# yakvrz/minesweeper-ppo

Hardware: AMD Instinct MI355X
Metric: env steps/sec (16x16x40, N envs) + PPO updates/sec at 1/2/4/8 MI355X (higher is better)
Workload: dtype u8/u64 board bits -> f32 obs; 1 GPU; board step 16x16x40, 4096 envs per GPU (BASELINE configs[1]); board=16x16x40, envs_per_gpu=4096, envs_total=4096, tape=0, parallelism=env-shard x1, no collective, obs_ring_slots=13

## Files before the change

### minesweeper-ppo_amd/csrc/msenv.hip

```cpp
#include <hip/hip_ext.h>
#include <hip/hip_runtime.h>

#include <stddef.h>
#include <stdint.h>
#include <stdio.h>
#include <stdlib.h>
#include <string.h>

#include <new>
#include <type_traits>
#include <vector>

#include "../../include/msenv.h"
#include "../../include/msenv_debug.h"
#include "msenv_internal.h"

namespace {

constexpr int kWave = 64;
constexpr int kMaxH = 64;
constexpr int kMaxW = 62;

struct alignas(16) EnvMeta {
  uint64_t st_hi, st_lo, inc_hi, inc_lo;
  uint32_t has32, uinteger;
  int32_t step_count;
  uint32_t flags;
};
static_assert(sizeof(EnvMeta) == 48, "EnvMeta layout");

struct KParams {
  const void* actions;
  float* obs;
  uint8_t* mask;
  float* reward;
  uint8_t* done;
  int32_t* step;
  int32_t* last_new;
  double* frac;
  int8_t* outcome;
  EnvMeta* meta;
  uint64_t* mine_words;
  uint64_t* rev_words;
  int64_t n;
  int32_t H, W, K, guarantee;
  int32_t actions_i32;
  double win_reward, loss_reward, step_penalty;
  const uint64_t* jump;
  uint64_t* diag;
  uint32_t dbg_flags;
  uint8_t* codes;
};

__device__ __forceinline__ int lane_id() { return __builtin_amdgcn_mbcnt_hi(~0u, __builtin_amdgcn_mbcnt_lo(~0u, 0u)); }

__device__ __forceinline__ uint32_t rfl(uint32_t x) { return (uint32_t)__builtin_amdgcn_readfirstlane((int)x); }
__device__ __forceinline__ uint64_t rfl64(uint64_t x) {
  return ((uint64_t)rfl((uint32_t)(x >> 32)) << 32) | rfl((uint32_t)x);
}

template <int CTRL>
__device__ __forceinline__ uint32_t dpp32(uint32_t v) {
  return (uint32_t)__builtin_amdgcn_update_dpp(0, (int)v, CTRL, 0xf, 0xf, true);
}
__device__ __forceinline__ uint64_t wave_shr1(uint64_t v) {
  return ((uint64_t)dpp32<0x138>((uint32_t)(v >> 32)) << 32) | dpp32<0x138>((uint32_t)v);
}
__device__ __forceinline__ uint64_t wave_shl1(uint64_t v) {
  return ((uint64_t)dpp32<0x130>((uint32_t)(v >> 32)) << 32) | dpp32<0x130>((uint32_t)v);
}
__device__ __forceinline__ uint32_t readlane32(uint32_t v, int l) {
  return (uint32_t)__builtin_amdgcn_readlane((int)v, l);
}
__device__ __forceinline__ uint64_t readlane64(uint64_t v, int l) {
  return ((uint64_t)readlane32((uint32_t)(v >> 32), l) << 32) | readlane32((uint32_t)v, l);
}
__device__ __forceinline__ void wave_sync() {
  __builtin_amdgcn_fence(__ATOMIC_RELEASE, "wavefront");
  __builtin_amdgcn_wave_barrier();
  __builtin_amdgcn_fence(__ATOMIC_ACQUIRE, "wavefront");
}
__device__ __forceinline__ uint32_t wave_sum(uint32_t v) {
  v += dpp32<0x111>(v);
  v += dpp32<0x112>(v);
  v += dpp32<0x114>(v);
  v += dpp32<0x118>(v);
  return readlane32(v, 15) + readlane32(v, 31) + readlane32(v, 47) + readlane32(v, 63);
}

#ifndef MS_OBS_STORE
#define MS_OBS_STORE 2
#endif
static_assert(MS_OBS_STORE >= 0 && MS_OBS_STORE <= 2, "MS_OBS_STORE: 0 plain, 1 nt, 2 write-through");
constexpr int kObsStore = MS_OBS_STORE;
constexpr int kObsStorePackedStep = kObsStore == 2 ? 1 : kObsStore;
constexpr int kObsStorePackedRun = kObsStore == 2 ? 0 : kObsStore;
typedef float f32x4_t __attribute__((ext_vector_type(4)));

template <int FORM = kObsStore>
__device__ __forceinline__ void store_plane4(float4* p, float4 v) {
  if constexpr (FORM == 1) {
    f32x4_t x = {v.x, v.y, v.z, v.w};
    __builtin_nontemporal_store(x, reinterpret_cast<f32x4_t*>(p));
  } else if constexpr (FORM == 2) {
    f32x4_t x = {v.x, v.y, v.z, v.w};
// ... 635 lines not shown
      }
      rev |= Fr;
      newly = (uint32_t)__popcll(Fr);
    }
  }
  const uint32_t packed = wave_sum(((uint32_t)__popcll(rev) << 16) | newly);
  total_rev = packed >> 16;
  newly = packed & 0xffffu;
  if (!cell_rev && outcome != MS_OUTCOME_LOSS && (int)total_rev >= A - p.K) {
    done = true;
    outcome = MS_OUTCOME_WIN;
  }
}

__device__ __forceinline__ void store_aux(const KParams& p, int64_t idx, int lane, double reward, bool done,
                                          int32_t step_count, uint32_t newly, uint32_t total_rev, int outcome, int A) {
  typedef __attribute__((address_space(1))) uint32_t gu32;
  typedef __attribute__((address_space(1))) uint8_t gu8;
  const uint64_t pr = rfl64((uint64_t)p.reward), ps = rfl64((uint64_t)p.step), pl = rfl64((uint64_t)p.last_new);
  const uint64_t pd = rfl64((uint64_t)p.done), po = rfl64((uint64_t)p.outcome);
  gu32* d4 = (gu32*)(lane == 0 ? pr : (lane == 1 ? ps : pl));
  const uint32_t v4 = lane == 0 ? __float_as_uint((float)reward) : (lane == 1 ? (uint32_t)step_count : newly);
  if (lane < 3 && d4) d4[idx] = v4;
  gu8* d1 = (gu8*)(lane == 0 ? pd : po);
  const uint8_t v1 = lane == 0 ? (uint8_t)(done ? 1 : 0) : (uint8_t)(int8_t)outcome;
  if (lane < 2 && d1) d1[idx] = v1;
  if (lane == 0 && p.frac) p.frac[idx] = (double)total_rev / (double)(A > 1 ? A : 1);
}

__device__ __forceinline__ void store_meta(EnvMeta* mp, const Pcg& rng, int32_t step_count, bool fc, int lane) {
  if (lane == 0) {
    *reinterpret_cast<ulonglong2*>(&mp->st_hi) = make_ulonglong2(rng.hi, rng.lo);
    *reinterpret_cast<uint4*>(&mp->has32) =
        make_uint4(rng.has32, rng.uinteger, (uint32_t)step_count, fc ? 1u : 0u);
  }
}

template <int H_, int W_, int EPW>
__global__ __launch_bounds__(64 * EPW) void k_step(EnvMeta* meta0, uint64_t* mine_words0, uint64_t* rev_words0,
                                                   const void* actions0, const uint64_t* jump0, int64_t n0,
                                                   int32_t actions_i32_0, int32_t K0, KParams p) {
  __shared__ uint64_t sR_all[EPW][kWave];
  __shared__ uint64_t sM_all[EPW][kWave + 2];
  __shared__ uint32_t sTab_all[EPW][(H_ && W_) ? H_ * W_ : kMaxH * kMaxW];
  const int lane = lane_id();
  const int wv = (EPW == 1) ? 0 : (int)rfl(threadIdx.x >> 6);
  const int64_t env_raw = (int64_t)blockIdx.x * EPW + wv;
  const bool live = env_raw < n0;
  const int64_t env = live ? env_raw : n0 - 1;
  uint64_t* sR = sR_all[wv];
  uint64_t* sM = sM_all[wv];
  uint32_t* sTab = sTab_all[wv];
  STAMP(0);
  const Geo<H_, W_> g(p.H, p.W);
  const int A = g.A(), NW = g.NW();

  EnvMeta* mp = meta0 + env;
  uint64_t* mwords = mine_words0 + env * NW;
  uint64_t* rwords = rev_words0 + env * NW;
  uint64_t mine = load_row(mwords, g, lane);
  uint64_t rev = load_row(rwords, g, lane);
  uint64_t J[4] = {0ull, 0ull, 0ull, 0ull};
  if (lane < K0) {
    const ulonglong2* e = reinterpret_cast<const ulonglong2*>(jump0 + 4 * lane);
    const ulonglong2 a0 = e[0], a1 = e[1];
    J[0] = a0.x;
    J[1] = a0.y;
    J[2] = a1.x;
    J[3] = a1.y;
  }
  Pcg rng;
  rng.hi = rfl64(mp->st_hi);
  rng.lo = rfl64(mp->st_lo);
  rng.ihi = rfl64(mp->inc_hi);
  rng.ilo = rfl64(mp->inc_lo);
  rng.has32 = rfl(mp->has32);
  rng.uinteger = rfl(mp->uinteger);
  int32_t step_count = (int32_t)rfl((uint32_t)mp->step_count);
  bool fc = (rfl(mp->flags) & 1u) != 0;
  const uint32_t* ap = reinterpret_cast<const uint32_t*>(actions0);
  const int64_t aw = actions_i32_0 ? env : 2 * env;
  const uint32_t a_lo = ap[aw], a_hi = ap[actions_i32_0 ? aw : aw + 1];
  int64_t a = actions_i32_0 ? (int64_t)(int32_t)a_lo : (int64_t)(((uint64_t)a_hi << 32) | a_lo);
  a = (int64_t)rfl64((uint64_t)a);
  int64_t cell64 = a % A;
  if (cell64 < 0) cell64 += A;
  const int cell = (int)cell64;
  if (!live) return;
  STAMP(1);

  double reward = 0.0;
  bool done = false;
  int outcome = MS_OUTCOME_NONE;
  uint32_t newly = 0, total_rev = 0;
  bool mines_changed = false;
  board_click(rng, mine, rev, fc, cell, p, J, sTab, sR, g, lane, done, outcome, newly, total_rev, mines_changed,
              env);
  STAMP(3);
  if (outcome == MS_OUTCOME_LOSS) reward += p.loss_reward;
  if (outcome == MS_OUTCOME_WIN) reward += p.win_reward;
  reward -= p.step_penalty;
  step_count += 1;

  store_aux(p, env, lane, reward, done, step_count, newly, total_rev, outcome, A);
  if (done) {
    mine = 0ull;
    rev = 0ull;
    fc = false;
    step_count = 0;
    mines_changed = true;
  }
  STAMP(4);

  if (p.obs || p.mask || p.codes) {
    stage_rows(sR, sM, rev, mine, g, lane);
    emit_obs(p.obs ? p.obs + env * 10 * A : nullptr, p.mask ? p.mask + env * A : nullptr,
             p.codes ? p.codes + env * A : nullptr, sR, sM, fc, g, lane, reinterpret_cast<uint8_t*>(sTab));
  }
  store_meta(mp, rng, step_count, fc, lane);
  if (mines_changed) store_rows(mwords, mine, sR, g, lane);
  store_rows(rwords, rev, sR, g, lane);
  STAMP(5);
}


template <int B>
__device__ __forceinline__ float ub2f(uint32_t w) {
  return (float)((w >> (8 * B)) & 0xffu);
}

__device__ __forceinline__ uint32_t row_shr1(uint32_t v) { return dpp32<0x111>(v); }
__device__ __forceinline__ uint32_t row_shl1(uint32_t v) { return dpp32<0x101>(v); }
template <int LPB>
__device__ __forceinline__ int board_base(int lane) { return lane & (64 - LPB); }
template <int LPB>
__device__ __forceinline__ uint32_t board_sum(uint32_t v, int lane) {
  v += dpp32<0x128>(v);
  v += dpp32<0x124>(v);
  v += dpp32<0x122>(v);
  v += dpp32<0x121>(v);
  if (LPB == 32) v += bperm(v, lane ^ 16);
  return v;
}
template <int LPB>
__device__ __forceinline__ bool board_any(bool v, int lane) {
  constexpr uint64_t M = LPB == 64 ? ~0ull : ((1ull << LPB) - 1ull);
  return ((__ballot(v) >> board_base<LPB>(lane)) & M) != 0ull;
}
template <int LPB>
__device__ __forceinline__ uint32_t board_read(uint32_t v, int lane, int r) {
  return bperm(v, board_base<LPB>(lane) | (r & 15));
}
template <int LPB>
__device__ __forceinline__ uint64_t board_read64(uint64_t v, int lane, int r) {
  return ((uint64_t)board_read<LPB>((uint32_t)(v >> 32), lane, r) << 32) | board_read<LPB>((uint32_t)v, lane, r);
}

template <int H_, int W_>
__device__ __forceinline__ uint32_t set_row(uint64_t s0, uint64_t s1, int r, const Geo<H_, W_>& g) {
  if (r >= g.H) return 0u;
  const int s = r * g.W;
  const uint64_t v = s >= 64 ? (s1 >> (s - 64)) : ((s0 >> s) | (s ? (s1 << (64 - s)) : 0ull));
  return (uint32_t)(v & g.rowmask());
}
__device__ __forceinline__ bool set_has(uint64_t s0, uint64_t s1, uint32_t c) {
  return (((c < 64u) ? s0 : s1) >> (c & 63u)) & 1ull;
}
__device__ __forceinline__ void set_add(uint64_t& s0, uint64_t& s1, uint32_t c) {
  const uint64_t bit = 1ull << (c & 63u);
  if (c < 64u) s0 |= bit;
  else s1 |= bit;
// ... 433 lines not shown
    const bool f = bperm(fc ? 1u : 0u, 16 * b) != 0u;
    const uint32_t m1 = m << 1, up1 = mu << 1, dn1 = md << 1;
    uint32_t cnt[4], rb[4];
#pragma unroll
    for (int e = 0; e < 4; ++e) {
      const int c = c0 + e;
      cnt[e] = (uint32_t)__popc((up1 >> c) & 7u) + (uint32_t)__popc((dn1 >> c) & 7u) + ((m1 >> c) & 1u) +
               ((m1 >> (c + 2)) & 1u);
      rb[e] = (rv >> c) & 1u;
    }
    if (ob) {
      float4* o4 = reinterpret_cast<float4*>(ob + (size_t)b * 10 * A) + lane;
#pragma unroll
      for (int ch = 0; ch < 10; ++ch) {
        float v[4];
#pragma unroll
        for (int e = 0; e < 4; ++e)
          v[e] = ch == 0 ? (float)rb[e] : ((f && rb[e] && cnt[e] + 1u == (uint32_t)ch) ? 1.f : 0.f);
        store_plane4(o4 + ch * (A / 4), make_float4(v[0], v[1], v[2], v[3]));
      }
    }
    if (mb)
      reinterpret_cast<uint32_t*>(mb + (size_t)b * A)[lane] =
          (rb[0] ^ 1u) | ((rb[1] ^ 1u) << 8) | ((rb[2] ^ 1u) << 16) | ((rb[3] ^ 1u) << 24);
  }
}

template <int H_, int W_, int BPW, int LPB, class Lds>
__device__ __forceinline__ void pk_store_state(EnvMeta* mp, uint64_t* mwords, uint64_t* rwords, const Pcg& rng,
                                               int32_t step_count, bool fc, uint32_t mine, uint32_t rev,
                                               bool mines_changed, bool live, Lds& S, int lane) {
  constexpr int RPW = 64 / W_;
  constexpr int NW = (H_ + RPW - 1) / RPW;
  const int r = lane & (LPB - 1);
  store_meta(mp, rng, step_count, fc, live ? r : 1);
  const int rb = board_base<LPB>(lane);
  S.row[lane] = mine;
  S.rev[lane] = rev;
  wave_sync();
  if (live && r < NW) {
    uint64_t am = 0ull, ar_ = 0ull;
#pragma unroll
    for (int k = 0; k < RPW; ++k)
      if (r * RPW + k < H_) {
        am |= (uint64_t)S.row[rb + r * RPW + k] << (k * W_);
        ar_ |= (uint64_t)S.rev[rb + r * RPW + k] << (k * W_);
      }
    if (mines_changed) mwords[r] = am;
    rwords[r] = ar_;
  }
}

template <int H_, int W_>
__device__ __forceinline__ void pk_load(const KParams& p, int64_t env, int r, uint32_t& mine, uint32_t& rev,
                                        uint64_t (&J)[4], Pcg& rng, int32_t& step_count, bool& fc) {
  constexpr int RPW = 64 / W_;
  constexpr int NW = (H_ + RPW - 1) / RPW;
  const Geo<H_, W_> g(H_, W_);
  const EnvMeta* mp = p.meta + env;
  mine = (uint32_t)load_row(p.mine_words + env * NW, g, r);
  rev = (uint32_t)load_row(p.rev_words + env * NW, g, r);
  J[0] = J[1] = J[2] = J[3] = 0ull;
  if (r < p.K) {
    const ulonglong2* e = reinterpret_cast<const ulonglong2*>(p.jump + 4 * r);
    const ulonglong2 a0 = e[0], a1 = e[1];
    J[0] = a0.x;
    J[1] = a0.y;
    J[2] = a1.x;
    J[3] = a1.y;
  }
  const ulonglong2 st = *reinterpret_cast<const ulonglong2*>(&mp->st_hi);
  const ulonglong2 inc = *reinterpret_cast<const ulonglong2*>(&mp->inc_hi);
  const uint4 m4 = *reinterpret_cast<const uint4*>(&mp->has32);
  rng.hi = st.x;
  rng.lo = st.y;
  rng.ihi = inc.x;
  rng.ilo = inc.y;
  rng.has32 = m4.x;
  rng.uinteger = m4.y;
  step_count = (int32_t)m4.z;
  fc = (m4.w & 1u) != 0;
}

template <int H_, int W_, int WPG, int BPW>
__global__ __launch_bounds__(64 * WPG) void k_step_packed(KParams p) {
  constexpr int LPB = kWave / BPW;
  constexpr bool BIG = packable16<H_, W_>();
  static_assert(BPW == 2 || BPW == 4, "boards per wave");
  static_assert(packable<H_, W_>() || (BIG && BPW == 4), "packed board shape");
  constexpr int A = H_ * W_;
  constexpr int RPW = 64 / W_;
  constexpr int NW = (H_ + RPW - 1) / RPW;
  using Lds = std::conditional_t<BIG, PackedLds16<H_, W_, BPW>, PackedLds<H_, W_, BPW>>;
  __shared__ Lds S_all[WPG];
  const int lane = lane_id();
  const int r = lane & (LPB - 1);
  const int wv = (WPG == 1) ? 0 : (int)rfl(threadIdx.x >> 6);
  Lds& S = S_all[wv];
  const int64_t env0 = ((int64_t)blockIdx.x * WPG + wv) * BPW;
  const bool wave_live = env0 < p.n;
  const int64_t env_raw = env0 + (lane / LPB);
  const bool live = env_raw < p.n;
  const int64_t env = live ? env_raw : p.n - 1;
  uint64_t* dgs = (p.diag && live) ? p.diag + env * 16 : nullptr;
  (void)dgs;
  DSTAMP(0);
  uint32_t mine, rev;
  uint64_t J[4];
  Pcg rng;
  int32_t step_count;
  bool fc;
  pk_load<H_, W_>(p, env, r, mine, rev, J, rng, step_count, fc);
  const uint32_t* ap = reinterpret_cast<const uint32_t*>(p.actions);
  const int64_t aw = p.actions_i32 ? env : 2 * env;
  const uint32_t a_lo = ap[aw], a_hi = ap[p.actions_i32 ? aw : aw + 1];
  if (!wave_live) return;
  const int64_t a = p.actions_i32 ? (int64_t)(int32_t)a_lo : (int64_t)(((uint64_t)a_hi << 32) | a_lo);
  int64_t cell64 = a % A;
  if (cell64 < 0) cell64 += A;
  DSTAMP(1);
  bool done, mines_changed = false, cell_rev;
  int outcome;
  uint32_t newly, total_rev;
  uint32_t* scr;
  if constexpr (BIG) scr = S.scr;
  else scr = S.row;
  pk_click<H_, W_, LPB>(p, rng, mine, rev, fc, (int)cell64, J, scr, lane, dgs, done, outcome, newly, total_rev,
                        mines_changed, cell_rev);
  DSTAMP(3);
  double reward = 0.0;
  if (outcome == MS_OUTCOME_LOSS) reward += p.loss_reward;
  if (outcome == MS_OUTCOME_WIN) reward += p.win_reward;
  reward -= p.step_penalty;
  step_count += 1;
  store_aux(p, env, live ? r : kWave, reward, done, step_count, newly, total_rev, outcome, A);
  if (done) {
    mine = 0u;
    rev = 0u;
    fc = false;
    step_count = 0;
    mines_changed = true;
  }
  DSTAMP(4);
  const int nbl = (p.n - env0 < BPW) ? (int)(p.n - env0) : BPW;
  if constexpr (BIG) {
    if (p.obs || p.mask)
      pk_emit16<H_, W_, BPW>(p.obs ? p.obs + env0 * 10 * A : nullptr, p.mask ? p.mask + env0 * A : nullptr, nbl, mine,
                             rev, fc, lane);
    DSTAMP(9);
  } else {
    if (p.obs || p.mask)
      pk_emit<H_, W_, BPW, LPB, kObsStorePackedStep>(p.obs ? p.obs + env0 * 10 * A : nullptr,
                                                     p.mask ? p.mask + env0 * A : nullptr, nbl, mine, rev, fc, S, lane,
                                                     dgs);
  }
  pk_store_state<H_, W_, BPW, LPB>(p.meta + env, p.mine_words + env * NW, p.rev_words + env * NW, rng, step_count, fc,
                                   mine, rev, mines_changed, live, S, lane);
  DSTAMP(5);
}

__global__ __launch_bounds__(256) void k_reset(EnvMeta* meta, uint64_t* mw, uint64_t* rw, int64_t n,
                                                int NW, float* obs, uint8_t* mask, int A) {
  const int64_t tid = (int64_t)blockIdx.x * blockDim.x + threadIdx.x;
  const int64_t nthreads = (int64_t)gridDim.x * blockDim.x;
  for (int64_t e = tid; e < n; e += nthreads) {
    meta[e].step_count = 0;
    meta[e].flags = 0;
  }
  for (int64_t i = tid; i < n * NW; i += nthreads) {
    mw[i] = 0;
    rw[i] = 0;
  }
  if (obs) {
    const int64_t tot = n * 10 * (int64_t)A;
    if ((tot & 3) == 0) {
      float4* o4 = reinterpret_cast<float4*>(obs);
      for (int64_t i = tid; i < tot / 4; i += nthreads) store_plane4(o4 + i, make_float4(0.f, 0.f, 0.f, 0.f));
    } else {
      for (int64_t i = tid; i < tot; i += nthreads) store_plane1(obs + i, 0.f);
    }
  }
  if (mask)
    for (int64_t i = tid; i < n * (int64_t)A; i += nthreads) mask[i] = 1;
}

__global__ __launch_bounds__(64) void k_labels(const EnvMeta* meta, const uint64_t* mw, const uint64_t* rw,
                                               int64_t n, int H, int W, float* labels, uint8_t* valid) {
  __shared__ uint64_t sMine[kWave], sRev[kWave];
  const int lane = lane_id();
  const int64_t env = blockIdx.x;
  if (env >= n) return;
  const Geo<0, 0> g(H, W);
  const int NW = g.NW(), A = g.A();
  sMine[lane] = load_row(mw + env * NW, g, lane);
  sRev[lane] = load_row(rw + env * NW, g, lane);
  const bool fc = (meta[env].flags & 1u) != 0;
  __syncthreads();
  for (int i = lane; i < A; i += kWave) {
    const int r = i / W, c = i - r * W;
    const uint32_t mb = (uint32_t)(sMine[r] >> c) & 1u, rb = (uint32_t)(sRev[r] >> c) & 1u;
    if (labels) labels[env * A + i] = fc ? (float)mb : 0.f;
    if (valid) valid[env * A + i] = fc ? (uint8_t)(rb ^ 1u) : 0;
  }
}

__global__ __launch_bounds__(64) void k_snapshot(const EnvMeta* meta, const uint64_t* mw, const uint64_t* rw,
                                                 int64_t n, int H, int W, uint8_t* mine, uint8_t* revealed,
                                                 uint8_t* counts, uint8_t* first_click, int32_t* step_count) {
  __shared__ uint64_t sMine[kWave + 2], sRev[kWave];
// ... 39 lines not shown

__device__ __forceinline__ uint32_t row_excl_scan16(uint32_t v) {
  uint32_t s = v;
  s += dpp32<0x111>(s);
  s += dpp32<0x112>(s);
  s += dpp32<0x114>(s);
  s += dpp32<0x118>(s);
  return s - v;
}

__device__ __forceinline__ uint32_t wave_excl_scan(uint32_t v) {
  uint32_t s = v;
  s += dpp32<0x111>(s);
  s += dpp32<0x112>(s);
  s += dpp32<0x114>(s);
  s += dpp32<0x118>(s);
  s += (uint32_t)__builtin_amdgcn_update_dpp(0, (int)s, 0x142, 0xa, 0xf, false);
  s += (uint32_t)__builtin_amdgcn_update_dpp(0, (int)s, 0x143, 0xc, 0xf, false);
  return s - v;
}

__device__ __forceinline__ int select_bit64(uint64_t x, uint32_t k) {
  int pos = 0;
#pragma unroll
  for (int half = 32; half >= 1; half >>= 1) {
    const uint64_t lowmask = (1ull << half) - 1ull;
    const uint32_t c = (uint32_t)__popcll(x & lowmask);
    if (k >= c) {
      k -= c;
      x >>= half;
      pos += half;
    }
  }
  return pos;
}

__device__ __forceinline__ int select_bit32(uint32_t x, uint32_t k) {
  int pos = 0;
#pragma unroll
  for (int half = 16; half >= 1; half >>= 1) {
    const uint32_t c = (uint32_t)__popc(x & ((1u << half) - 1u));
    if (k >= c) {
      k -= c;
      x >>= half;
      pos += half;
    }
  }
  return pos;
}

__device__ __forceinline__ uint32_t mod64_small(uint64_t x, uint32_t c) {
  const uint32_t hi = (uint32_t)(x >> 32), lo = (uint32_t)x;
  const uint32_t r = ((hi % c) * ((0u - c) % c)) % c;
  return (r + lo % c) % c;
}

template <int H_, int W_>
__global__ __launch_bounds__(64) void k_tape(const uint64_t* mw, const uint64_t* rw, int64_t n, int H_rt, int W_rt,
                                             int64_t env_begin, uint64_t t, int mode, int64_t* actions) {
  const int64_t env = (int64_t)blockIdx.x * 64 + threadIdx.x;
  if (env >= n) return;
  const Geo<H_, W_> g(H_rt, W_rt);
  const int W = g.W, rpw = g.RPW(), NW = g.NW();
  constexpr int kNW = (H_ && W_) ? (H_ + (64 / W_) - 1) / (64 / W_) : 64;
  constexpr bool kStatic = H_ && W_;
  const bool safe_mode = mode == MS_TAPE_SAFE_BIASED;
  const uint64_t* rp = rw + env * NW;
  const uint64_t* mp = mw + env * NW;
  auto valid_mask = [&](int w) -> uint64_t {
    const int rows = min(rpw, g.H - w * rpw);
    const int bits = rows * W;
    return bits >= 64 ? ~0ull : ((1ull << bits) - 1ull);
  };
  uint64_t vw[kStatic ? kNW : 1], sw[kStatic ? kNW : 1];
  uint32_t n_valid = 0, n_safe = 0;
  if constexpr (kStatic) {
    uint64_t rr[kNW], mm[kNW];
#pragma unroll
    for (int w = 0; w < kNW; ++w) rr[w] = rp[w];
    if (safe_mode) {
#pragma unroll
      for (int w = 0; w < kNW; ++w) mm[w] = mp[w];
    }
#pragma unroll
    for (int w = 0; w < kNW; ++w) {
      vw[w] = ~rr[w] & valid_mask(w);
      n_valid += (uint32_t)__popcll(vw[w]);
      sw[w] = safe_mode ? (vw[w] & ~mm[w]) : 0ull;
      n_safe += (uint32_t)__popcll(sw[w]);
    }
  } else {
    for (int w = 0; w < NW; ++w) {
      const uint64_t v = ~rp[w] & valid_mask(w);
      n_valid += (uint32_t)__popcll(v);
      if (safe_mode) n_safe += (uint32_t)__popcll(v & ~mp[w]);
    }
  }
  const uint64_t gidx = (uint64_t)(env_begin + env);
  const uint64_t x = splitmix64(0xC0FFEEull ^ (gidx << 32) ^ t);
  const bool want_safe = safe_mode && (x & 0xFFFFull) < 65208ull && n_safe > 0;
  const uint32_t cnt = want_safe ? n_safe : n_valid;
  const uint64_t sel = safe_mode ? (x >> 16) : x;
  int64_t act = 0;
  if (cnt > 0) {
    uint32_t target = mod64_small(sel, cnt);
    if constexpr (kStatic) {
#pragma unroll
      for (int w = 0; w < kNW; ++w) {
        if (target != 0xFFFFFFFFu) {
          const uint64_t b = want_safe ? sw[w] : vw[w];
          const uint32_t pc = (uint32_t)__popcll(b);
          if (target < pc) {
            const int pos = select_bit64(b, target);
            const int r = w * rpw + pos / W;
            act = (int64_t)r * W + (pos - (pos / W) * W);
            target = 0xFFFFFFFFu;
          } else {
            target -= pc;
          }
        }
      }
    } else {
      for (int w = 0; w < NW && target != 0xFFFFFFFFu; ++w) {
        uint64_t b = ~rp[w] & valid_mask(w);
        if (want_safe) b &= ~mp[w];
        const uint32_t pc = (uint32_t)__popcll(b);
        if (target < pc) {
          const int pos = select_bit64(b, target);
          const int r = w * rpw + pos / W;
          act = (int64_t)r * W + (pos - (pos / W) * W);
          target = 0xFFFFFFFFu;
        } else {
          target -= pc;
        }
      }
    }
  }
  actions[env] = act;
}

struct LateCfg {
  double prob;
  int32_t min_hidden, max_hidden, max_attempts, max_extra_steps;
};

__device__ __forceinline__ Pcg keyed_late_pcg(uint64_t seed, uint64_t gidx, uint64_t st_hi, uint64_t st_lo) {
  Pcg L;
  L.hi = splitmix64(seed ^ splitmix64(gidx ^ 0x6C8E9CF570932BD5ull));
  L.lo = splitmix64(L.hi ^ st_lo);
  L.ihi = splitmix64(L.lo ^ st_hi);
  L.ilo = splitmix64(L.ihi ^ 0xA0761D6478BD642Full) | 1ull;
  L.has32 = 0u;
  L.uinteger = 0u;
  return L;
}

struct LateState {
  uint64_t mine, rev;
  uint64_t st_hi, st_lo, inc_hi, inc_lo;
  uint32_t has32, uinteger, step_count, flags;
};

template <int H_, int W_>
__device__ __forceinline__ LateState late_load(const KParams& p, int64_t env, const Geo<H_, W_>& g, int lane) {
  const int NW = g.NW();
  const EnvMeta* mp = p.meta + env;
  LateState s;
  s.mine = load_row(p.mine_words + env * NW, g, lane);
  s.rev = load_row(p.rev_words + env * NW, g, lane);
  s.st_hi = rfl64(mp->st_hi);
  s.st_lo = rfl64(mp->st_lo);
  s.inc_hi = rfl64(mp->inc_hi);
  s.inc_lo = rfl64(mp->inc_lo);
  s.has32 = rfl(mp->has32);
  s.uinteger = rfl(mp->uinteger);
  s.step_count = rfl((uint32_t)mp->step_count);
  s.flags = rfl(mp->flags);
  return s;
}

struct LateRng {
  Pcg base;
  uint32_t xlo, xhi;
// ... 457 lines not shown
  const int r = lane & (LPB - 1);
  const uint32_t valid = ~rev & ROWMASK & (r < H_ ? ~0u : 0u);
  const uint64_t x = splitmix64(0xC0FFEEull ^ (gidx << 32) ^ t);
  uint32_t bits = valid;
  uint32_t cnt = board_sum<LPB>((uint32_t)__popc(valid), lane);
  uint64_t sel = x;
  if (mode == MS_TAPE_SAFE_BIASED) {
    const uint32_t safe = valid & ~mine;
    const uint32_t n_safe = board_sum<LPB>((uint32_t)__popc(safe), lane);
    sel = x >> 16;
    if ((x & 0xFFFFull) < 65208ull && n_safe > 0) {
      bits = safe;
      cnt = n_safe;
    }
  }
  const uint32_t target = mod64_small(sel, cnt ? cnt : 1u);
  const uint32_t pc = (uint32_t)__popc(bits);
  const uint32_t before = row_excl_scan(pc);
  const bool hit = target >= before && target < before + pc;
  const uint64_t who = (__ballot(hit) >> board_base<LPB>(lane)) & BM;
  const int src = who ? __ffsll((unsigned long long)who) - 1 : 0;
  const int col = (int)board_read<LPB>(hit ? (uint32_t)select_bit64(bits, target - before) : 0u, lane, src);
  return cnt ? src * W_ + col : 0;
}

template <int H_, int W_, int WPG, int BPW>
__global__ __launch_bounds__(64 * WPG) void k_run_packed(KParams p, RunParams rp) {
  constexpr int LPB = kWave / BPW;
  constexpr bool BIG = packable16<H_, W_>();
  static_assert(BPW == 2 || BPW == 4, "boards per wave");
  static_assert(packable<H_, W_>() || (BIG && BPW == 4), "packed board shape");
  constexpr int A = H_ * W_;
  constexpr int RPW = 64 / W_;
  constexpr int NW = (H_ + RPW - 1) / RPW;
  using Lds = std::conditional_t<BIG, PackedLds16<H_, W_, BPW>, PackedLds<H_, W_, BPW>>;
  __shared__ Lds S_all[WPG];
  const int lane = lane_id();
  const int r = lane & (LPB - 1);
  const int wv = (WPG == 1) ? 0 : (int)rfl(threadIdx.x >> 6);
  Lds& S = S_all[wv];
  uint32_t* scr;
  if constexpr (BIG) scr = S.scr;
  else scr = S.row;
  const int64_t env0 = ((int64_t)blockIdx.x * WPG + wv) * BPW;
  if (env0 >= p.n) return;
  const int64_t env_raw = env0 + (lane / LPB);
  const bool live = env_raw < p.n;
  const int64_t env = live ? env_raw : p.n - 1;
  uint32_t mine, rev;
  uint64_t J[4];
  Pcg rng;
  int32_t step_count;
  bool fc;
  pk_load<H_, W_>(p, env, r, mine, rev, J, rng, step_count, fc);
  const uint64_t gidx = (uint64_t)(rp.env_begin + env);
  const int64_t n = p.n;
  const int nbl = (n - env0 < BPW) ? (int)(n - env0) : BPW;
  for (int t = 0; t < rp.T; ++t) {
    const int64_t sbase = rp.slots ? (int64_t)t * n : 0;
    const int cell = pk_tape_cell<H_, W_, LPB>(mine, rev, lane, gidx, rp.t0 + (uint64_t)t, rp.mode);
    bool done, mines_changed = false, cell_rev;
    int outcome;
    uint32_t newly, total_rev;
    pk_click<H_, W_, LPB>(p, rng, mine, rev, fc, cell, J, scr, lane, nullptr, done, outcome, newly, total_rev,
                          mines_changed, cell_rev);
    double reward = 0.0;
    if (outcome == MS_OUTCOME_LOSS) reward += p.loss_reward;
    if (outcome == MS_OUTCOME_WIN) reward += p.win_reward;
    reward -= p.step_penalty;
    step_count += 1;
    if (rp.actions && live && r == 0) rp.actions[sbase + env] = cell;
    store_aux(p, sbase + env, live ? r : kWave, reward, done, step_count, newly, total_rev, outcome, A);
    if (done) {
      mine = 0u;
      rev = 0u;
      fc = false;
      step_count = 0;
    }
    if constexpr (BIG) {
      if (p.obs || p.mask)
        pk_emit16<H_, W_, BPW>(p.obs ? p.obs + (sbase + env0) * 10 * A : nullptr,
                               p.mask ? p.mask + (sbase + env0) * A : nullptr, nbl, mine, rev, fc, lane);
    } else {
      if (p.obs || p.mask)
        pk_emit<H_, W_, BPW, LPB, kObsStorePackedRun>(p.obs ? p.obs + (sbase + env0) * 10 * A : nullptr,
                                                      p.mask ? p.mask + (sbase + env0) * A : nullptr, nbl, mine, rev,
                                                      fc, S, lane, nullptr);
    }
    wave_sync();
  }
  pk_store_state<H_, W_, BPW, LPB>(p.meta + env, p.mine_words + env * NW, p.rev_words + env * NW, rng, step_count, fc,
                                   mine, rev, true, live, S, lane);
}

__global__ __launch_bounds__(256) void k_gae(const float* __restrict__ rewards, const float* __restrict__ values,
                                             const uint8_t* __restrict__ dones, const float* __restrict__ last_values,
                                             int T, int64_t N, float gamma, float gl, float* __restrict__ adv,
                                             float* __restrict__ ret) {
#pragma clang fp contract(off)
  const int64_t n = (int64_t)blockIdx.x * blockDim.x + threadIdx.x;
  if (n >= N) return;
  float last_adv = 0.f;
  float nv = last_values[n];
  for (int t = T - 1; t >= 0; --t) {
    const int64_t i = (int64_t)t * N + n;
    const float v = values[i];
    const float nnt = 1.0f - (dones[i] ? 1.0f : 0.0f);
// ... 174 lines not shown
  if (left < excl) {
    const uint32_t thr = (0xffffffffu - j) % excl;
    while (left < thr) {
      m = (uint64_t)host_next32(r) * excl;
      left = (uint32_t)m;
    }
  }
  return (uint32_t)(m >> 32);
}

}

struct ms_handle {
  ms_cfg cfg;
  int64_t n_total, env_begin, n;
  int H, W, A, NW;
  int device;
  EnvMeta* meta;
  uint64_t* mine_words;
  uint64_t* rev_words;
  uint64_t* jump;
  uint64_t* diag;
  uint32_t dbg_flags;
  int epw;
  int late_on;
  hipEvent_t ev_start, ev_stop;
  LateCfg late;
  Pcg* late_rng;
  int late_mode;
  uint64_t late_seed;
  int32_t avoid_budget;
  int32_t posterior_budget;
};

namespace {

bool shape_ok(const ms_cfg* c) {
  return c->H >= 1 && c->H <= kMaxH && c->W >= 1 && c->W <= kMaxW && c->mine_count >= 0 &&
         c->mine_count < c->H * c->W;
}

constexpr int64_t kPack16MinEnvs = 65536;
constexpr int64_t kPack16RunMinEnvs = 0;

template <int H_, int W_>
void launch_step(const KParams& p, int epw, hipStream_t s, hipEvent_t ev0, hipEvent_t ev1) {
  if constexpr (packable16<H_, W_>()) {
    if (p.K >= 1 && p.K <= 48 &&
        !(p.dbg_flags & (MS_DBG_ONE_BOARD_PER_WAVE | MS_DBG_FORCE_CHAIN_PLACEMENT | MS_DBG_TWO_BOARDS_PER_WAVE)) &&
        (p.n >= kPack16MinEnvs || (p.dbg_flags & MS_DBG_FORCE_PACKED)) && ((uintptr_t)p.obs & 15u) == 0 &&
        ((uintptr_t)p.mask & 3u) == 0 && !p.codes) {
      constexpr int WPG = 4;
      const unsigned grid = (unsigned)((p.n + 4 * WPG - 1) / (4 * WPG));
      hipExtLaunchKernelGGL((k_step_packed<H_, W_, WPG, 4>), dim3(grid), dim3(64 * WPG), 0, s, ev0, ev1, 0, p);
      return;
    }
  }
  if constexpr (packable<H_, W_>()) {
    if (p.K >= 1 && p.K <= 16 && !(p.dbg_flags & (MS_DBG_ONE_BOARD_PER_WAVE | MS_DBG_FORCE_CHAIN_PLACEMENT)) &&
        ((uintptr_t)p.obs & 15u) == 0 && ((uintptr_t)p.mask & 3u) == 0 && !p.codes) {
      constexpr int WPG = 4;
      if (p.dbg_flags & MS_DBG_TWO_BOARDS_PER_WAVE) {
        const unsigned grid = (unsigned)((p.n + 2 * WPG - 1) / (2 * WPG));
        hipExtLaunchKernelGGL((k_step_packed<H_, W_, WPG, 2>), dim3(grid), dim3(64 * WPG), 0, s, ev0, ev1, 0, p);
      } else {
        const unsigned grid = (unsigned)((p.n + 4 * WPG - 1) / (4 * WPG));
        hipExtLaunchKernelGGL((k_step_packed<H_, W_, WPG, 4>), dim3(grid), dim3(64 * WPG), 0, s, ev0, ev1, 0, p);
      }
      return;
    }
  }
  if (H_ && W_ && epw == 4) {
    hipExtLaunchKernelGGL((k_step<H_, W_, 4>), dim3((unsigned)((p.n + 3) / 4)), dim3(256), 0, s, ev0, ev1, 0, p.meta,
                          p.mine_words, p.rev_words, p.actions, p.jump, p.n, p.actions_i32, p.K, p);
  } else {
    hipExtLaunchKernelGGL((k_step<H_, W_, 1>), dim3((unsigned)p.n), dim3(64), 0, s, ev0, ev1, 0, p.meta, p.mine_words,
                          p.rev_words, p.actions, p.jump, p.n, p.actions_i32, p.K, p);
  }
}

template <int H_, int W_>
void launch_run(const KParams& p, const RunParams& r, hipStream_t s, hipEvent_t ev0, hipEvent_t ev1) {
  if constexpr (packable16<H_, W_>()) {
    if (p.K >= 1 && p.K <= 48 &&
        !(p.dbg_flags & (MS_DBG_ONE_BOARD_PER_WAVE | MS_DBG_FORCE_CHAIN_PLACEMENT | MS_DBG_TWO_BOARDS_PER_WAVE)) &&
        (p.n >= kPack16RunMinEnvs || (p.dbg_flags & MS_DBG_FORCE_PACKED)) && ((uintptr_t)p.obs & 15u) == 0 &&
        ((uintptr_t)p.mask & 3u) == 0) {
      constexpr int WPG = 4;
      const unsigned grid = (unsigned)((p.n + 4 * WPG - 1) / (4 * WPG));
      hipExtLaunchKernelGGL((k_run_packed<H_, W_, WPG, 4>), dim3(grid), dim3(64 * WPG), 0, s, ev0, ev1, 0, p, r);
      return;
    }
  }
  if constexpr (packable<H_, W_>()) {
    const bool slot_ok = !r.slots || ((p.n * H_ * W_) & 3) == 0;
    if (p.K >= 1 && p.K <= 16 && !(p.dbg_flags & (MS_DBG_ONE_BOARD_PER_WAVE | MS_DBG_FORCE_CHAIN_PLACEMENT)) &&
        ((uintptr_t)p.obs & 15u) == 0 && ((uintptr_t)p.mask & 3u) == 0 && slot_ok) {
      constexpr int WPG = 4;
      if (p.dbg_flags & MS_DBG_TWO_BOARDS_PER_WAVE) {
        const unsigned grid = (unsigned)((p.n + 2 * WPG - 1) / (2 * WPG));
        hipExtLaunchKernelGGL((k_run_packed<H_, W_, WPG, 2>), dim3(grid), dim3(64 * WPG), 0, s, ev0, ev1, 0, p, r);
      } else {
        const unsigned grid = (unsigned)((p.n + 4 * WPG - 1) / (4 * WPG));
        hipExtLaunchKernelGGL((k_run_packed<H_, W_, WPG, 4>), dim3(grid), dim3(64 * WPG), 0, s, ev0, ev1, 0, p, r);
      }
      return;
    }
  }
  if (H_ && W_)
    hipExtLaunchKernelGGL((k_run<H_, W_, 4>), dim3((unsigned)((p.n + 3) / 4)), dim3(256), 0, s, ev0, ev1, 0, p, r);
  else hipExtLaunchKernelGGL((k_run<H_, W_, 1>), dim3((unsigned)p.n), dim3(64), 0, s, ev0, ev1, 0, p, r);
}

template <int H_, int W_>
void launch_late_t(const KParams& p, Pcg* st, const LateCfg& c, const uint8_t* need, hipStream_t s) {
  hipLaunchKernelGGL((k_late<H_, W_>), dim3(1), dim3(64), 0, s, p, st, c, need);
}

void fill_params(const ms_handle* h, KParams& p) {
  p.meta = h->meta;
// ... 317 lines not shown
  p.step = step;
  p.last_new = last_new;
  p.frac = revealed_frac;
  p.outcome = outcome;
  RunParams r;
  r.t0 = t0;
  r.T = T;
  r.mode = mode;
  r.slots = slots ? 1 : 0;
  r.env_begin = h->env_begin;
  r.actions = actions;
  const hipStream_t s = (hipStream_t)stream;
  if (h->H == 16 && h->W == 16) launch_run<16, 16>(p, r, s, h->ev_start, h->ev_stop);
  else if (h->H == 9 && h->W == 9) launch_run<9, 9>(p, r, s, h->ev_start, h->ev_stop);
  else if (h->H == 30 && h->W == 16) launch_run<30, 16>(p, r, s, h->ev_start, h->ev_stop);
  else if (h->H == 16 && h->W == 30) launch_run<16, 30>(p, r, s, h->ev_start, h->ev_stop);
  else if (h->H == 8 && h->W == 8) launch_run<8, 8>(p, r, s, h->ev_start, h->ev_stop);
  else launch_run<0, 0>(p, r, s, h->ev_start, h->ev_stop);
  hipError_t e = hipGetLastError();
  return e == hipSuccess ? MS_OK : hip_fail(e, "ms_run_tape launch");
}

int ms_labels(ms_handle* h, float* mine_labels, uint8_t* mine_valid, void* stream) {
  if (!h) return fail(MS_EINVAL, "ms_labels: null handle");
  hipLaunchKernelGGL(k_labels, dim3((unsigned)h->n), dim3(64), 0, (hipStream_t)stream, h->meta, h->mine_words,
                     h->rev_words, h->n, h->H, h->W, mine_labels, mine_valid);
  hipError_t e = hipGetLastError();
  return e == hipSuccess ? MS_OK : hip_fail(e, "ms_labels launch");
}

int ms_snapshot(ms_handle* h, uint8_t* mine, uint8_t* revealed, uint8_t* counts, uint8_t* first_click,
                int32_t* step_count, void* stream) {
  if (!h) return fail(MS_EINVAL, "ms_snapshot: null handle");
  hipLaunchKernelGGL(k_snapshot, dim3((unsigned)h->n), dim3(64), 0, (hipStream_t)stream, h->meta,
                     h->mine_words, h->rev_words, h->n, h->H, h->W, mine, revealed, counts, first_click,
                     step_count);
  hipError_t e = hipGetLastError();
  return e == hipSuccess ? MS_OK : hip_fail(e, "ms_snapshot launch");
}

int ms_rng_state(ms_handle* h, uint64_t* out, void* stream) {
  if (!h || !out) return fail(MS_EINVAL, "ms_rng_state: null argument");
  hipLaunchKernelGGL(k_rng_state, dim3((unsigned)((h->n + 255) / 256)), dim3(256), 0, (hipStream_t)stream,
                     h->meta, h->n, out);
  hipError_t e = hipGetLastError();
  return e == hipSuccess ? MS_OK : hip_fail(e, "ms_rng_state launch");
}

int ms_tape_actions(ms_handle* h, uint64_t t, int32_t mode, int64_t* actions, void* stream) {
  if (!h || !actions) return fail(MS_EINVAL, "ms_tape_actions: null argument");
  if (mode != MS_TAPE_UNIFORM && mode != MS_TAPE_SAFE_BIASED) return fail(MS_EINVAL, "ms_tape_actions: bad mode");
  const hipStream_t s = (hipStream_t)stream;
  const dim3 grid((unsigned)((h->n + 63) / 64)), block(64);
  if (h->H == 16 && h->W == 16)
    hipLaunchKernelGGL((k_tape<16, 16>), grid, block, 0, s, h->mine_words, h->rev_words, h->n, h->H, h->W,
                       h->env_begin, t, mode, actions);
  else if (h->H == 9 && h->W == 9)
    hipLaunchKernelGGL((k_tape<9, 9>), grid, block, 0, s, h->mine_words, h->rev_words, h->n, h->H, h->W,
                       h->env_begin, t, mode, actions);
  else if (h->H == 30 && h->W == 16)
    hipLaunchKernelGGL((k_tape<30, 16>), grid, block, 0, s, h->mine_words, h->rev_words, h->n, h->H, h->W,
                       h->env_begin, t, mode, actions);
  else if (h->H == 16 && h->W == 30)
    hipLaunchKernelGGL((k_tape<16, 30>), grid, block, 0, s, h->mine_words, h->rev_words, h->n, h->H, h->W,
                       h->env_begin, t, mode, actions);
  else
    hipLaunchKernelGGL((k_tape<0, 0>), grid, block, 0, s, h->mine_words, h->rev_words, h->n, h->H, h->W,
                       h->env_begin, t, mode, actions);
  hipError_t e = hipGetLastError();
  return e == hipSuccess ? MS_OK : hip_fail(e, "ms_tape_actions launch");
}

int ms_gae(const float* rewards, const float* values, const uint8_t* dones, const float* last_values, int32_t T,
           int64_t N, float gamma, float gamma_lambda, float* adv, float* ret, void* stream) {
  if (!rewards || !values || !dones || !last_values || !adv || !ret || T <= 0 || N <= 0)
    return fail(MS_EINVAL, "ms_gae: bad argument");
  hipLaunchKernelGGL(k_gae, dim3((unsigned)((N + 255) / 256)), dim3(256), 0, (hipStream_t)stream, rewards, values,
                     dones, last_values, (int)T, N, gamma, gamma_lambda, adv, ret);
  hipError_t e = hipGetLastError();
  return e == hipSuccess ? MS_OK : hip_fail(e, "ms_gae launch");
}

int ms_sample_masked(const float* logits, const uint8_t* mask, int64_t N, int32_t A, int64_t row_begin,
                     uint64_t seed, uint64_t counter, int64_t* actions, float* logp, void* stream) {
  if (!logits || !mask || !actions || !logp || N <= 0 || A <= 0 || row_begin < 0)
    return fail(MS_EINVAL, "ms_sample_masked: bad argument");
  hipLaunchKernelGGL(k_sample, dim3((unsigned)((N + 3) / 4)), dim3(256), 0, (hipStream_t)stream, logits, mask, N,
                     (int)A, row_begin, seed, counter, actions, logp);
  hipError_t e = hipGetLastError();
  return e == hipSuccess ? MS_OK : hip_fail(e, "ms_sample_masked launch");
}

int ms_dropout_masks(const int64_t* rows, int64_t N, int32_t nblk, int32_t C, uint64_t seed, uint64_t counter,
                     float p, float* out, void* stream) {
  if (!rows || !out || N <= 0 || nblk <= 0 || C <= 0 || (C & 3) || !(p > 0.f && p < 1.f))
    return fail(MS_EINVAL, "ms_dropout_masks: bad argument");
  const int64_t total = (int64_t)nblk * N * (C / 4);
  const unsigned grid = (unsigned)std::min<int64_t>((total + 255) / 256, 8192);
  hipLaunchKernelGGL(k_dropout, dim3(grid), dim3(256), 0, (hipStream_t)stream, rows, N, (int)nblk, (int)C, seed,
                     counter, p, 1.0f / (1.0f - p), out);
  hipError_t e = hipGetLastError();
  return e == hipSuccess ? MS_OK : hip_fail(e, "ms_dropout_masks launch");
}

}
```

Measured before the change: 356.7 million env_steps/s.

## Pass hot step pointers as scalar kernel args, warm KParams lines, rework tape kernel

The packed step kernel now takes the meta, board-word, action and jump pointers plus n and K as direct kernel arguments instead of reading them from the large KParams struct. The one-board kernel touches one dword in each 64-byte line of KParams early, so the later scalar loads hit cache. It also moves the aux store after observation emission. The tape kernel gets a branchless word-select path, a cheaper final modulo and a smaller argument list. The aim is to cut kernarg and scalar-load latency at kernel start. The cost is more launch arguments and empty asm constraints that could limit scheduling.

Measured after the change: 370.2 million env_steps/s, median of 6. +3.8%, better.

```diff
diff --git a/minesweeper-ppo_amd/csrc/msenv.hip b/minesweeper-ppo_amd/csrc/msenv.hip
--- a/minesweeper-ppo_amd/csrc/msenv.hip
+++ b/minesweeper-ppo_amd/csrc/msenv.hip
@@ -51,6 +51,31 @@
   uint32_t dbg_flags;
   uint8_t* codes;
 };
+
+struct KParamsWarm {
+  uint32_t w[5];
+};
+__device__ __forceinline__ uint32_t kparams_dword(const void* field) {
+  return *reinterpret_cast<const uint32_t*>(field);
+}
+__device__ __forceinline__ KParamsWarm kparams_warm(const KParams& p) {
+  static_assert(offsetof(KParams, outcome) - offsetof(KParams, obs) < 64 &&
+                    offsetof(KParams, guarantee) - offsetof(KParams, outcome) < 64 &&
+                    offsetof(KParams, step_penalty) - offsetof(KParams, guarantee) < 64 &&
+                    offsetof(KParams, codes) - offsetof(KParams, step_penalty) < 64 &&
+                    sizeof(KParams) - offsetof(KParams, codes) <= 8,
+                "kparams_warm: one touch per 64-byte line");
+  KParamsWarm k;
+  k.w[0] = kparams_dword(&p.obs);
+  k.w[1] = kparams_dword(&p.outcome);
+  k.w[2] = kparams_dword(&p.guarantee);
+  k.w[3] = kparams_dword(&p.step_penalty);
+  k.w[4] = kparams_dword(&p.codes);
+  return k;
+}
+__device__ __forceinline__ void kparams_warm_wait(const KParamsWarm& k) {
+  asm volatile("" ::"s"(k.w[0]), "s"(k.w[1]), "s"(k.w[2]), "s"(k.w[3]), "s"(k.w[4]));
+}
 
 __device__ __forceinline__ int lane_id() { return __builtin_amdgcn_mbcnt_hi(~0u, __builtin_amdgcn_mbcnt_lo(~0u, 0u)); }
 
@@ -792,6 +817,7 @@
   uint64_t* sM = sM_all[wv];
   uint32_t* sTab = sTab_all[wv];
   STAMP(0);
+  const KParamsWarm warm = kparams_warm(p);
   const Geo<H_, W_> g(p.H, p.W);
   const int A = g.A(), NW = g.NW();
 
@@ -826,6 +852,7 @@
   int64_t cell64 = a % A;
   if (cell64 < 0) cell64 += A;
   const int cell = (int)cell64;
+  kparams_warm_wait(warm);
   if (!live) return;
   STAMP(1);
 
@@ -841,8 +868,7 @@
   if (outcome == MS_OUTCOME_WIN) reward += p.win_reward;
   reward -= p.step_penalty;
   step_count += 1;
-
-  store_aux(p, env, lane, reward, done, step_count, newly, total_rev, outcome, A);
+  const int32_t step_out = step_count;
   if (done) {
     mine = 0ull;
     rev = 0ull;
@@ -857,6 +883,7 @@
     emit_obs(p.obs ? p.obs + env * 10 * A : nullptr, p.mask ? p.mask + env * A : nullptr,
              p.codes ? p.codes + env * A : nullptr, sR, sM, fc, g, lane, reinterpret_cast<uint8_t*>(sTab));
   }
+  store_aux(p, env, lane, reward, done, step_out, newly, total_rev, outcome, A);
   store_meta(mp, rng, step_count, fc, lane);
   if (mines_changed) store_rows(mwords, mine, sR, g, lane);
   store_rows(rwords, rev, sR, g, lane);
@@ -1396,17 +1423,18 @@
 }
 
 template <int H_, int W_>
-__device__ __forceinline__ void pk_load(const KParams& p, int64_t env, int r, uint32_t& mine, uint32_t& rev,
+__device__ __forceinline__ void pk_load(const EnvMeta* meta, const uint64_t* mine_words, const uint64_t* rev_words,
+                                        const uint64_t* jump, int K, int64_t env, int r, uint32_t& mine, uint32_t& rev,
                                         uint64_t (&J)[4], Pcg& rng, int32_t& step_count, bool& fc) {
   constexpr int RPW = 64 / W_;
   constexpr int NW = (H_ + RPW - 1) / RPW;
   const Geo<H_, W_> g(H_, W_);
-  const EnvMeta* mp = p.meta + env;
-  mine = (uint32_t)load_row(p.mine_words + env * NW, g, r);
-  rev = (uint32_t)load_row(p.rev_words + env * NW, g, r);
+  const EnvMeta* mp = meta + env;
+  mine = (uint32_t)load_row(mine_words + env * NW, g, r);
+  rev = (uint32_t)load_row(rev_words + env * NW, g, r);
   J[0] = J[1] = J[2] = J[3] = 0ull;
-  if (r < p.K) {
-    const ulonglong2* e = reinterpret_cast<const ulonglong2*>(p.jump + 4 * r);
+  if (r < K) {
+    const ulonglong2* e = reinterpret_cast<const ulonglong2*>(jump + 4 * r);
     const ulonglong2 a0 = e[0], a1 = e[1];
     J[0] = a0.x;
     J[1] = a0.y;
@@ -1427,7 +1455,9 @@
 }
 
 template <int H_, int W_, int WPG, int BPW>
-__global__ __launch_bounds__(64 * WPG) void k_step_packed(KParams p) {
+__global__ __launch_bounds__(64 * WPG) void k_step_packed(EnvMeta* meta0, uint64_t* mine_words0, uint64_t* rev_words0,
+                                                          const void* actions0, const uint64_t* jump0, int64_t n0,
+                                                          int32_t actions_i32_0, int32_t K0, KParams p) {
   constexpr int LPB = kWave / BPW;
   constexpr bool BIG = packable16<H_, W_>();
   static_assert(BPW == 2 || BPW == 4, "boards per wave");
@@ -1442,10 +1472,10 @@
   const int wv = (WPG == 1) ? 0 : (int)rfl(threadIdx.x >> 6);
   Lds& S = S_all[wv];
   const int64_t env0 = ((int64_t)blockIdx.x * WPG + wv) * BPW;
-  const bool wave_live = env0 < p.n;
+  const bool wave_live = env0 < n0;
   const int64_t env_raw = env0 + (lane / LPB);
-  const bool live = env_raw < p.n;
-  const int64_t env = live ? env_raw : p.n - 1;
+  const bool live = env_raw < n0;
+  const int64_t env = live ? env_raw : n0 - 1;
   uint64_t* dgs = (p.diag && live) ? p.diag + env * 16 : nullptr;
   (void)dgs;
   DSTAMP(0);
@@ -1454,12 +1484,12 @@
   Pcg rng;
   int32_t step_count;
   bool fc;
-  pk_load<H_, W_>(p, env, r, mine, rev, J, rng, step_count, fc);
-  const uint32_t* ap = reinterpret_cast<const uint32_t*>(p.actions);
-  const int64_t aw = p.actions_i32 ? env : 2 * env;
-  const uint32_t a_lo = ap[aw], a_hi = ap[p.actions_i32 ? aw : aw + 1];
+  pk_load<H_, W_>(meta0, mine_words0, rev_words0, jump0, K0, env, r, mine, rev, J, rng, step_count, fc);
+  const uint32_t* ap = reinterpret_cast<const uint32_t*>(actions0);
+  const int64_t aw = actions_i32_0 ? env : 2 * env;
+  const uint32_t a_lo = ap[aw], a_hi = ap[actions_i32_0 ? aw : aw + 1];
   if (!wave_live) return;
-  const int64_t a = p.actions_i32 ? (int64_t)(int32_t)a_lo : (int64_t)(((uint64_t)a_hi << 32) | a_lo);
+  const int64_t a = actions_i32_0 ? (int64_t)(int32_t)a_lo : (int64_t)(((uint64_t)a_hi << 32) | a_lo);
   int64_t cell64 = a % A;
   if (cell64 < 0) cell64 += A;
   DSTAMP(1);
@@ -1486,7 +1516,7 @@
     mines_changed = true;
   }
   DSTAMP(4);
-  const int nbl = (p.n - env0 < BPW) ? (int)(p.n - env0) : BPW;
+  const int nbl = (n0 - env0 < BPW) ? (int)(n0 - env0) : BPW;
   if constexpr (BIG) {
     if (p.obs || p.mask)
       pk_emit16<H_, W_, BPW>(p.obs ? p.obs + env0 * 10 * A : nullptr, p.mask ? p.mask + env0 * A : nullptr, nbl, mine,
@@ -1498,7 +1528,7 @@
                                                      p.mask ? p.mask + env0 * A : nullptr, nbl, mine, rev, fc, S, lane,
                                                      dgs);
   }
-  pk_store_state<H_, W_, BPW, LPB>(p.meta + env, p.mine_words + env * NW, p.rev_words + env * NW, rng, step_count, fc,
+  pk_store_state<H_, W_, BPW, LPB>(meta0 + env, mine_words0 + env * NW, rev_words0 + env * NW, rng, step_count, fc,
                                    mine, rev, mines_changed, live, S, lane);
   DSTAMP(5);
 }
@@ -1644,15 +1674,20 @@
 __device__ __forceinline__ uint32_t mod64_small(uint64_t x, uint32_t c) {
   const uint32_t hi = (uint32_t)(x >> 32), lo = (uint32_t)x;
   const uint32_t r = ((hi % c) * ((0u - c) % c)) % c;
-  return (r + lo % c) % c;
+  const uint32_t s = r + lo % c;
+  return s >= c ? s - c : s;
+}
+
+__device__ __forceinline__ void tape_tie(uint64_t& word, uint64_t x) {
+  asm volatile("" : "+v"(word) : "v"(x));
 }
 
 template <int H_, int W_>
-__global__ __launch_bounds__(64) void k_tape(const uint64_t* mw, const uint64_t* rw, int64_t n, int H_rt, int W_rt,
-                                             int64_t env_begin, uint64_t t, int mode, int64_t* actions) {
+__global__ __launch_bounds__(64) void k_tape(const uint64_t* mw, const uint64_t* rw, int64_t* actions, int64_t n,
+                                             int64_t env_begin, uint64_t t, int mode, uint32_t hw) {
   const int64_t env = (int64_t)blockIdx.x * 64 + threadIdx.x;
   if (env >= n) return;
-  const Geo<H_, W_> g(H_rt, W_rt);
+  const Geo<H_, W_> g((int)(hw & 0xffffu), (int)(hw >> 16));
   const int W = g.W, rpw = g.RPW(), NW = g.NW();
   constexpr int kNW = (H_ && W_) ? (H_ + (64 / W_) - 1) / (64 / W_) : 64;
   constexpr bool kStatic = H_ && W_;
@@ -1664,63 +1699,73 @@
     const int bits = rows * W;
     return bits >= 64 ? ~0ull : ((1ull << bits) - 1ull);
   };
-  uint64_t vw[kStatic ? kNW : 1], sw[kStatic ? kNW : 1];
-  uint32_t n_valid = 0, n_safe = 0;
+  const uint64_t gidx = (uint64_t)(env_begin + env);
+  int64_t act = 0;
   if constexpr (kStatic) {
-    uint64_t rr[kNW], mm[kNW];
-#pragma unroll
-    for (int w = 0; w < kNW; ++w) rr[w] = rp[w];
+    uint64_t b[kNW], mm[kNW];
+#pragma unroll
+    for (int w = 0; w < kNW; ++w) b[w] = rp[w];
     if (safe_mode) {
 #pragma unroll
       for (int w = 0; w < kNW; ++w) mm[w] = mp[w];
     }
+    const uint64_t x = splitmix64(0xC0FFEEull ^ (gidx << 32) ^ t);
+#pragma unroll
+    for (int w = 0; w < kNW; ++w) tape_tie(b[w], x);
+    uint32_t cnt = 0;
 #pragma unroll
     for (int w = 0; w < kNW; ++w) {
-      vw[w] = ~rr[w] & valid_mask(w);
-      n_valid += (uint32_t)__popcll(vw[w]);
-      sw[w] = safe_mode ? (vw[w] & ~mm[w]) : 0ull;
-      n_safe += (uint32_t)__popcll(sw[w]);
-    }
+      b[w] = ~b[w] & valid_mask(w);
+      cnt += (uint32_t)__popcll(b[w]);
+    }
+    uint64_t sel = x;
+    if (safe_mode) {
+      uint64_t sw[kNW];
+      uint32_t n_safe = 0;
+#pragma unroll
+      for (int w = 0; w < kNW; ++w) {
+        sw[w] = b[w] & ~mm[w];
+        n_safe += (uint32_t)__popcll(sw[w]);
+      }
+      sel = x >> 16;
+      if ((x & 0xFFFFull) < 65208ull && n_safe > 0) {
+        cnt = n_safe;
+#pragma unroll
+        for (int w = 0; w < kNW; ++w) b[w] = sw[w];
+      }
+    }
+    const uint32_t target = mod64_small(sel, cnt ? cnt : 1u);
+    uint64_t bw = b[0];
+    uint32_t before = 0, acc = (uint32_t)__popcll(b[0]);
+    int base = 0;
+#pragma unroll
+    for (int w = 1; w < kNW; ++w) {
+      const bool here = target >= acc;
+      bw = here ? b[w] : bw;
+      before = here ? acc : before;
+      base = here ? w * rpw * W : base;
+      acc += (uint32_t)__popcll(b[w]);
+    }
+    if (cnt > 0) act = (int64_t)(base + select_bit64(bw, target - before));
   } else {
+    uint32_t n_valid = 0, n_safe = 0;
     for (int w = 0; w < NW; ++w) {
       const uint64_t v = ~rp[w] & valid_mask(w);
       n_valid += (uint32_t)__popcll(v);
       if (safe_mode) n_safe += (uint32_t)__popcll(v & ~mp[w]);
     }
-  }
-  const uint64_t gidx = (uint64_t)(env_begin + env);
-  const uint64_t x = splitmix64(0xC0FFEEull ^ (gidx << 32) ^ t);
-  const bool want_safe = safe_mode && (x & 0xFFFFull) < 65208ull && n_safe > 0;
-  const uint32_t cnt = want_safe ? n_safe : n_valid;
-  const uint64_t sel = safe_mode ? (x >> 16) : x;
-  int64_t act = 0;
-  if (cnt > 0) {
-    uint32_t target = mod64_small(sel, cnt);
-    if constexpr (kStatic) {
-#pragma unroll
-      for (int w = 0; w < kNW; ++w) {
-        if (target != 0xFFFFFFFFu) {
-          const uint64_t b = want_safe ? sw[w] : vw[w];
-          const uint32_t pc = (uint32_t)__popcll(b);
-          if (target < pc) {
-            const int pos = select_bit64(b, target);
-            const int r = w * rpw + pos / W;
-            act = (int64_t)r * W + (pos - (pos / W) * W);
-            target = 0xFFFFFFFFu;
-          } else {
-            target -= pc;
-          }
-        }
-      }
-    } else {
+    const uint64_t x = splitmix64(0xC0FFEEull ^ (gidx << 32) ^ t);
+    const bool want_safe = safe_mode && (x & 0xFFFFull) < 65208ull && n_safe > 0;
+    const uint32_t cnt = want_safe ? n_safe : n_valid;
+    const uint64_t sel = safe_mode ? (x >> 16) : x;
+    if (cnt > 0) {
+      uint32_t target = mod64_small(sel, cnt);
       for (int w = 0; w < NW && target != 0xFFFFFFFFu; ++w) {
         uint64_t b = ~rp[w] & valid_mask(w);
         if (want_safe) b &= ~mp[w];
         const uint32_t pc = (uint32_t)__popcll(b);
         if (target < pc) {
-          const int pos = select_bit64(b, target);
-          const int r = w * rpw + pos / W;
-          act = (int64_t)r * W + (pos - (pos / W) * W);
+          act = (int64_t)(w * rpw * W + select_bit64(b, target));
           target = 0xFFFFFFFFu;
         } else {
           target -= pc;
@@ -2284,7 +2329,7 @@
   Pcg rng;
   int32_t step_count;
   bool fc;
-  pk_load<H_, W_>(p, env, r, mine, rev, J, rng, step_count, fc);
+  pk_load<H_, W_>(p.meta, p.mine_words, p.rev_words, p.jump, p.K, env, r, mine, rev, J, rng, step_count, fc);
   const uint64_t gidx = (uint64_t)(rp.env_begin + env);
   const int64_t n = p.n;
   const int nbl = (n - env0 < BPW) ? (int)(n - env0) : BPW;
@@ -2565,7 +2610,8 @@
         ((uintptr_t)p.mask & 3u) == 0 && !p.codes) {
       constexpr int WPG = 4;
       const unsigned grid = (unsigned)((p.n + 4 * WPG - 1) / (4 * WPG));
-      hipExtLaunchKernelGGL((k_step_packed<H_, W_, WPG, 4>), dim3(grid), dim3(64 * WPG), 0, s, ev0, ev1, 0, p);
+      hipExtLaunchKernelGGL((k_step_packed<H_, W_, WPG, 4>), dim3(grid), dim3(64 * WPG), 0, s, ev0, ev1, 0, p.meta,
+                            p.mine_words, p.rev_words, p.actions, p.jump, p.n, p.actions_i32, p.K, p);
       return;
     }
   }
@@ -2575,10 +2621,12 @@
       constexpr int WPG = 4;
       if (p.dbg_flags & MS_DBG_TWO_BOARDS_PER_WAVE) {
         const unsigned grid = (unsigned)((p.n + 2 * WPG - 1) / (2 * WPG));
-        hipExtLaunchKernelGGL((k_step_packed<H_, W_, WPG, 2>), dim3(grid), dim3(64 * WPG), 0, s, ev0, ev1, 0, p);
+        hipExtLaunchKernelGGL((k_step_packed<H_, W_, WPG, 2>), dim3(grid), dim3(64 * WPG), 0, s, ev0, ev1, 0, p.meta,
+                            p.mine_words, p.rev_words, p.actions, p.jump, p.n, p.actions_i32, p.K, p);
       } else {
         const unsigned grid = (unsigned)((p.n + 4 * WPG - 1) / (4 * WPG));
-        hipExtLaunchKernelGGL((k_step_packed<H_, W_, WPG, 4>), dim3(grid), dim3(64 * WPG), 0, s, ev0, ev1, 0, p);
+        hipExtLaunchKernelGGL((k_step_packed<H_, W_, WPG, 4>), dim3(grid), dim3(64 * WPG), 0, s, ev0, ev1, 0, p.meta,
+                            p.mine_words, p.rev_words, p.actions, p.jump, p.n, p.actions_i32, p.K, p);
       }
       return;
     }
@@ -3002,21 +3050,22 @@
   if (mode != MS_TAPE_UNIFORM && mode != MS_TAPE_SAFE_BIASED) return fail(MS_EINVAL, "ms_tape_actions: bad mode");
   const hipStream_t s = (hipStream_t)stream;
   const dim3 grid((unsigned)((h->n + 63) / 64)), block(64);
+  const uint32_t hw = (uint32_t)h->H | ((uint32_t)h->W << 16);
   if (h->H == 16 && h->W == 16)
-    hipLaunchKernelGGL((k_tape<16, 16>), grid, block, 0, s, h->mine_words, h->rev_words, h->n, h->H, h->W,
-                       h->env_begin, t, mode, actions);
+    hipLaunchKernelGGL((k_tape<16, 16>), grid, block, 0, s, h->mine_words, h->rev_words, actions, h->n,
+                       h->env_begin, t, mode, hw);
   else if (h->H == 9 && h->W == 9)
-    hipLaunchKernelGGL((k_tape<9, 9>), grid, block, 0, s, h->mine_words, h->rev_words, h->n, h->H, h->W,
-                       h->env_begin, t, mode, actions);
+    hipLaunchKernelGGL((k_tape<9, 9>), grid, block, 0, s, h->mine_words, h->rev_words, actions, h->n,
+                       h->env_begin, t, mode, hw);
   else if (h->H == 30 && h->W == 16)
-    hipLaunchKernelGGL((k_tape<30, 16>), grid, block, 0, s, h->mine_words, h->rev_words, h->n, h->H, h->W,
-                       h->env_begin, t, mode, actions);
+    hipLaunchKernelGGL((k_tape<30, 16>), grid, block, 0, s, h->mine_words, h->rev_words, actions, h->n,
+                       h->env_begin, t, mode, hw);
   else if (h->H == 16 && h->W == 30)
-    hipLaunchKernelGGL((k_tape<16, 30>), grid, block, 0, s, h->mine_words, h->rev_words, h->n, h->H, h->W,
-                       h->env_begin, t, mode, actions);
+    hipLaunchKernelGGL((k_tape<16, 30>), grid, block, 0, s, h->mine_words, h->rev_words, actions, h->n,
+                       h->env_begin, t, mode, hw);
   else
-    hipLaunchKernelGGL((k_tape<0, 0>), grid, block, 0, s, h->mine_words, h->rev_words, h->n, h->H, h->W,
-                       h->env_begin, t, mode, actions);
+    hipLaunchKernelGGL((k_tape<0, 0>), grid, block, 0, s, h->mine_words, h->rev_words, actions, h->n,
+                       h->env_begin, t, mode, hw);
   hipError_t e = hipGetLastError();
   return e == hipSuccess ? MS_OK : hip_fail(e, "ms_tape_actions launch");
 }
```
